# johnomotani/SharedMemSparseLU.jl

Measured on AMD Instinct MI355X. Metric: nnz(L+U)/s + achieved HBM GB/s, 3D Poisson 128³ numeric LU, 1/2/4/8 GPU, higher is better.
Workload: dtype f64

## Files before the change

### sharedmemsparselu.jl_amd/csrc/kernels_gemm.hip

```cpp
#include "kernels_common.hpp"

namespace smlu {

__device__ __forceinline__ int find_gemm_task(const GemmTask* __restrict__ t, int cnt, int64_t b) {
  int lo = 0, hi = cnt - 1;
  while (lo < hi) {
    int mid = (lo + hi + 1) >> 1;
    if (t[mid].tile0 <= b) lo = mid;
    else hi = mid - 1;
  }
  return lo;
}


__device__ __forceinline__ int64_t xcd_remap(int64_t b, int64_t nwg) {
  const int64_t q = nwg >> 3, r = nwg & 7, x = b & 7;
  return (x < r ? x * (q + 1) : r * (q + 1) + (x - r) * q) + (b >> 3);
}
__device__ __forceinline__ int64_t xcd_window_remap(int64_t b, int64_t nwg) {
  constexpr int64_t W = 512;
  if (b >= (nwg / W) * W) return b;
  const int64_t w0 = b - b % W, i = b % W;
  return w0 + (i & 7) * (W / 8) + (i >> 3);
}
template <int TS>
__device__ __forceinline__ void tile_rc(const GemmTask& t, int64_t tl, int& tm, int& tn) {
  constexpr int GM = 8;
  const int64_t tiles_n = (t.n + TS - 1) / TS;
  const int64_t g = tl / (GM * tiles_n);
  const int first = (int)(g * GM);
  const int gm = min(GM, t.tiles_m - first);
  const int64_t in = tl - g * GM * tiles_n;
  tm = first + (int)(in % gm);
  tn = (int)(in / gm);
}

struct GrowthArgs {
  int32_t* info;
  double* growth;
  double piv_tol;
};
__device__ __forceinline__ void tile_growth(const GrowthArgs& ga, int sid, double g) {
  g = wave_max(g);
  if ((threadIdx.x & 63) == 0 && g > 0.0) {
    atomic_max_pos(&ga.growth[0], g);
    if (g > 1.0 / ga.piv_tol) atomicOr(&ga.info[sid], 2);
  }
}

#define GBM 64
#define GBN 64
#define GBK 16
template <bool TRSM>
__global__ __launch_bounds__(256) void k_gemm(const GemmTask* __restrict__ tasks, int ntask, GrowthArgs ga) {
  __shared__ double As[2][GBK][GBM + 2];
  __shared__ double Bs[2][GBK][GBN + 2];
  const int64_t b = xcd_remap(blockIdx.x, gridDim.x);
  const GemmTask t = tasks[find_gemm_task(tasks, ntask, b)];
  const gdbl* gA = gbl(t.A);
  const gdbl* gB = gbl(t.B);
  gdbl* gC = gbl(t.C);
  int tm, tn;
  tile_rc<GBM>(t, b - t.tile0, tm, tn);
  const int m0 = tm * GBM, n0 = tn * GBN;
  const int tid = threadIdx.x;
  const int tx = tid & 15, ty = tid >> 4;
  double acc[4][4];
#pragma unroll
  for (int j = 0; j < 4; ++j) {
    const int col = n0 + ty + 16 * j;
#pragma unroll
    for (int i = 0; i < 4; ++i) {
      const int row = m0 + tx + 16 * i;
      acc[i][j] = (col < t.n && row < t.m) ? gC[(int64_t)col * t.ldc + row] : 0.0;
    }
  }
  const int ar = tid & 63, ak = tid >> 6;
  const int bk = tid & 15, bc = tid >> 4;
  double ra[4], rb[4];
  const int K = t.k;
  auto gload = [&](int k0) {
#pragma unroll
    for (int r = 0; r < 4; ++r) {
      int kk = ak + 4 * r;
      int row = m0 + ar;
      ra[r] = (row < t.m && k0 + kk < K) ? gA[(int64_t)(k0 + kk) * t.lda + row] : 0.0;
      int col = n0 + bc + 16 * r;
      rb[r] = (col < t.n && k0 + bk < K) ? gB[(int64_t)col * t.ldb + k0 + bk] : 0.0;
    }
  };
  auto sstore = [&](int buf) {
#pragma unroll
    for (int r = 0; r < 4; ++r) {
      As[buf][ak + 4 * r][ar] = ra[r];
      Bs[buf][bk][bc + 16 * r] = -rb[r];
    }
  };
  int nk = (K + GBK - 1) / GBK;
  gload(0);
  sstore(0);
  __syncthreads();
  for (int kt = 0; kt < nk; ++kt) {
    const int cur = kt & 1;
    if (kt + 1 < nk) gload((kt + 1) * GBK);
#pragma unroll 4
    for (int kk = 0; kk < GBK; ++kk) {
      double a[4], bb[4];
#pragma unroll
      for (int i = 0; i < 4; ++i) a[i] = As[cur][kk][tx + 16 * i];
#pragma unroll
      for (int j = 0; j < 4; ++j) bb[j] = Bs[cur][kk][ty + 16 * j];
#pragma unroll
      for (int i = 0; i < 4; ++i)
#pragma unroll
        for (int j = 0; j < 4; ++j) acc[i][j] = fma(a[i], bb[j], acc[i][j]);
    }
    if (kt + 1 < nk) sstore(cur ^ 1);
    __syncthreads();
  }
  double gmax = 0.0;
#pragma unroll
  for (int j = 0; j < 4; ++j) {
    const int col = n0 + ty + 16 * j;
#pragma unroll
    for (int i = 0; i < 4; ++i) {
      const int row = m0 + tx + 16 * i;
      if (col < t.n && row < t.m) {
        gC[(int64_t)col * t.ldc + row] = acc[i][j];
        gmax = fmax(gmax, fabs(acc[i][j]));
      }
    }
  }
  if (TRSM && t.gsid >= 0) tile_growth(ga, t.gsid, gmax);
}

typedef double v4d __attribute__((ext_vector_type(4)));
template <bool TRSM>
__global__ __launch_bounds__(256) void k_gemm64_mfma(const GemmTask* __restrict__ tasks, int ntask, GrowthArgs ga) {
  __shared__ double As[2][GBK][GBM + 2];
  __shared__ double Bs[2][GBK][GBN + 2];
  const int64_t b = xcd_remap(blockIdx.x, gridDim.x);
  const GemmTask t = tasks[find_gemm_task(tasks, ntask, b)];
  const gdbl* gA = gbl(t.A);
  const gdbl* gB = gbl(t.B);
  gdbl* gC = gbl(t.C);
  int tm, tn;
  tile_rc<GBM>(t, b - t.tile0, tm, tn);
  const int m0 = tm * GBM, n0 = tn * GBN;
  const int tid = threadIdx.x, lane = tid & 63;
  const int wv = __builtin_amdgcn_readfirstlane(tid >> 6);
  const int wr = (wv & 1) * 32, wc = (wv >> 1) * 32;
  const int li = lane & 15, lk = lane >> 4;
  v4d acc[2][2];
#pragma unroll
  for (int i = 0; i < 2; ++i) {
    const int row = m0 + wr + 16 * i + li;
#pragma unroll
    for (int j = 0; j < 2; ++j)
#pragma unroll
      for (int r = 0; r < 4; ++r) {
        const int col = n0 + wc + 16 * j + lk + 4 * r;
        acc[i][j][r] = (col < t.n && row < t.m) ? gC[(int64_t)col * t.ldc + row] : 0.0;
      }
  }
  const int ar = tid & 63, ak = tid >> 6;
  const int bk = tid & 15, bc = tid >> 4;
  double ra[4], rb[4];
  const int K = t.k;
  auto gload = [&](int k0) {
#pragma unroll
    for (int r = 0; r < 4; ++r) {
      const int kk = ak + 4 * r;
      const int row = m0 + ar;
      ra[r] = (row < t.m && k0 + kk < K) ? gA[(int64_t)(k0 + kk) * t.lda + row] : 0.0;
      const int col = n0 + bc + 16 * r;
      rb[r] = (col < t.n && k0 + bk < K) ? gB[(int64_t)col * t.ldb + k0 + bk] : 0.0;
    }
  };
  auto sstore = [&](int buf) {
#pragma unroll
    for (int r = 0; r < 4; ++r) {
      As[buf][ak + 4 * r][ar] = ra[r];
      Bs[buf][bk][bc + 16 * r] = -rb[r];
    }
  };
  const int nk = (K + GBK - 1) / GBK;
  gload(0);
  sstore(0);
  __syncthreads();
  for (int kt = 0; kt < nk; ++kt) {
    const int cur = kt & 1;
    if (kt + 1 < nk) gload((kt + 1) * GBK);
#pragma unroll
    for (int kq = 0; kq < GBK / 4; ++kq) {
      const int k = 4 * kq + lk;
      double fa[2], fb[2];
#pragma unroll
      for (int i = 0; i < 2; ++i) fa[i] = As[cur][k][wr + 16 * i + li];
#pragma unroll
      for (int j = 0; j < 2; ++j) fb[j] = Bs[cur][k][wc + 16 * j + li];
#pragma unroll
      for (int i = 0; i < 2; ++i)
#pragma unroll
        for (int j = 0; j < 2; ++j) acc[i][j] = __builtin_amdgcn_mfma_f64_16x16x4f64(fb[j], fa[i], acc[i][j], 0, 0, 0);
    }
    if (kt + 1 < nk) sstore(cur ^ 1);
    __syncthreads();
  }
  double gmax = 0.0;
#pragma unroll
  for (int i = 0; i < 2; ++i) {
    const int row = m0 + wr + 16 * i + li;
#pragma unroll
    for (int j = 0; j < 2; ++j)
#pragma unroll
      for (int r = 0; r < 4; ++r) {
        const int col = n0 + wc + 16 * j + lk + 4 * r;
        if (col < t.n && row < t.m) {
          gC[(int64_t)col * t.ldc + row] = acc[i][j][r];
          gmax = fmax(gmax, fabs(acc[i][j][r]));
        }
      }
  }
  if (TRSM && t.gsid >= 0) tile_growth(ga, t.gsid, gmax);
}

__device__ __forceinline__ double k64_tile_mfma(const gdbl* gA, int lda, const gdbl* gB, int ldb, gdbl* gC, int ldc,
                                                int m, int n, int K, int m0, int n0,
                                                double (&As)[64][GBM + 2], double (&Bs)[64][GBN + 2]) {
  const int tid = threadIdx.x, lane = tid & 63;
  const int wv = __builtin_amdgcn_readfirstlane(tid >> 6);
  const int wr = (wv & 1) * 32, wc = (wv >> 1) * 32;
  const int li = lane & 15, lk = lane >> 4;
  v4d acc[2][2];
#pragma unroll
  for (int i = 0; i < 2; ++i) {
    const int row = m0 + wr + 16 * i + li;
#pragma unroll
    for (int j = 0; j < 2; ++j)
#pragma unroll
      for (int r = 0; r < 4; ++r) {
        const int col = n0 + wc + 16 * j + lk + 4 * r;
        acc[i][j][r] = (col < n && row < m) ? gC[(int64_t)col * ldc + row] : 0.0;
      }
  }
  const int ar = tid & 63, ak = tid >> 6;
  double ra[16], rb[16];
#pragma unroll
  for (int r = 0; r < 16; ++r) {
    const int kk = ak + 4 * r, row = m0 + ar;
    ra[r] = (row < m && kk < K) ? gA[(int64_t)kk * lda + row] : 0.0;
    const int col = n0 + ak + 4 * r;
    rb[r] = (col < n && ar < K) ? gB[(int64_t)col * ldb + ar] : 0.0;
  }
#pragma unroll
  for (int r = 0; r < 16; ++r) {
    As[ak + 4 * r][ar] = ra[r];
    Bs[ar][ak + 4 * r] = -rb[r];
  }
  __syncthreads();
  auto kquad = [&](int kq) {
    const int k = 4 * kq + lk;
    double fa[2], fb[2];
#pragma unroll
    for (int i = 0; i < 2; ++i) fa[i] = As[k][wr + 16 * i + li];
#pragma unroll
    for (int j = 0; j < 2; ++j) fb[j] = Bs[k][wc + 16 * j + li];
#pragma unroll
    for (int i = 0; i < 2; ++i)
#pragma unroll
      for (int j = 0; j < 2; ++j) acc[i][j] = __builtin_amdgcn_mfma_f64_16x16x4f64(fb[j], fa[i], acc[i][j], 0, 0, 0);
  };
  if (K == 64) {
#pragma unroll
    for (int kq = 0; kq < 16; ++kq) kquad(kq);
  } else {
    const int nkq = (K + 3) >> 2;
    for (int kq = 0; kq < nkq; ++kq) kquad(kq);
  }
  double gmax = 0.0;
#pragma unroll
  for (int i = 0; i < 2; ++i) {
    const int row = m0 + wr + 16 * i + li;
#pragma unroll
    for (int j = 0; j < 2; ++j)
#pragma unroll
      for (int r = 0; r < 4; ++r) {
        const int col = n0 + wc + 16 * j + lk + 4 * r;
        if (col < n && row < m) {
          gC[(int64_t)col * ldc + row] = acc[i][j][r];
          gmax = fmax(gmax, fabs(acc[i][j][r]));
        }
      }
  }
  return gmax;
}

template <bool TRSM>
__global__ __launch_bounds__(256) void k_gemm_k64(const GemmTask* __restrict__ tasks, int ntask, GrowthArgs ga) {
  __shared__ double As[64][GBM + 2];
  __shared__ double Bs[64][GBN + 2];
  const int64_t b = xcd_remap(blockIdx.x, gridDim.x);
  const GemmTask t = tasks[find_gemm_task(tasks, ntask, b)];
  int tm, tn;
  tile_rc<GBM>(t, b - t.tile0, tm, tn);
  const double gmax = k64_tile_mfma(gbl(t.A), t.lda, gbl(t.B), t.ldb, gbl(t.C), t.ldc, t.m, t.n, t.k, tm * GBM,
                                    tn * GBN, As, Bs);
  if (TRSM && t.gsid >= 0) tile_growth(ga, t.gsid, gmax);
}

#define HBM_ 128
#define HBK_ 16
#define HLDB_ (HBM_ + 2)
__device__ __forceinline__ double sel0(bool c, double x) {
  return __longlong_as_double(__double_as_longlong(x) & (c ? -1LL : 0LL));
}
struct GatherArgs {
  const F22Gather* tg;
  const F22Child* ch;
  const int32_t* inv;
  const double* scratch;
};
struct F22Tile {
  const F22Child* ch;
  const int32_t* inv;
  const double* scratch;
  int cnt;
};
__device__ __forceinline__ double f22_child_val(const char* src, int nuc, int ri, int cj) {
  const bool ok = (ri | cj) >= 0;
  const uint32_t off = ok ? ((uint32_t)cj * (uint32_t)nuc + (uint32_t)ri) * 8u : 0u;
  return sel0(ok, *(const gdbl*)(src + off));
}
__device__ __forceinline__ void f22_child_add(v4d (&acc)[4][4], int j, const char* src, int nuc, const int (&ri)[4],
                                              const int (&cj)[4]) {
  double v[4][4];
#pragma unroll
  for (int r = 0; r < 4; ++r)
#pragma unroll
    for (int i = 0; i < 4; ++i) v[i][r] = f22_child_val(src, nuc, ri[i], cj[r]);
#pragma unroll
  for (int r = 0; r < 4; ++r)
#pragma unroll
    for (int i = 0; i < 4; ++i) acc[i][j][r] += v[i][r];
  __builtin_amdgcn_sched_barrier(0);
}
template <bool TRSM, bool FULL, bool GATHER = false>
__device__ __forceinline__ void gemm128_mfma_body(const GemmTask& t, int m0, int n0,
                                                double (&As)[2][HBK_][HBM_], double (&Bs)[2][HBK_][HLDB_],
                                                const GrowthArgs& ga, const F22Tile& fg = F22Tile{}) {
  const gdbl* gA = gbl(t.A);
  const gdbl* gB = gbl(t.B);
  gdbl* gC = gbl(t.C);
  const int tid = threadIdx.x, lane = tid & 63, wv = tid >> 6;
  const int wr = (wv & 1) * 64, wc = (wv >> 1) * 64;
  const int li = lane & 15, lk = lane >> 4;
  v4d acc[4][4];
  if (GATHER && fg.cnt >= 0) {
#pragma unroll
    for (int i = 0; i < 4; ++i)
#pragma unroll
      for (int j = 0; j < 4; ++j) acc[i][j] = v4d{0.0, 0.0, 0.0, 0.0};
#pragma unroll 1
    for (int d = 0; d < fg.cnt; ++d) {
      const F22Child c = fg.ch[d];
      if (c.hi < m0 + wr || c.lo >= m0 + wr + 64 || c.hi < n0 + wc || c.lo >= n0 + wc + 64) continue;
      const int32_t* inv = fg.inv + c.inv;
      const char* src = reinterpret_cast<const char*>(fg.scratch + c.foff);
      int ri[4], cj[4][4];
#pragma unroll
      for (int i = 0; i < 4; ++i) {
        const int row = m0 + wr + 16 * i + li;
        const int v = inv[min(row, t.m - 1)];
        ri[i] = row < t.m ? v : -1;
      }
#pragma unroll
      for (int j = 0; j < 4; ++j)
#pragma unroll
        for (int r = 0; r < 4; ++r) {
          const int col = n0 + wc + 16 * j + lk + 4 * r;
          const int v = inv[min(col, t.n - 1)];
          cj[j][r] = col < t.n ? v : -1;
        }
      __builtin_amdgcn_sched_barrier(0);
#pragma unroll
      for (int j = 0; j < 4; ++j) f22_child_add(acc, j, src, c.nu, ri, cj[j]);
    }
  } else {
#pragma unroll
    for (int i = 0; i < 4; ++i) {
      const int row = m0 + wr + 16 * i + li;
#pragma unroll
      for (int j = 0; j < 4; ++j)
#pragma unroll
        for (int r = 0; r < 4; ++r) {
          const int col = n0 + wc + 16 * j + lk + 4 * r;
          acc[i][j][r] = (FULL || (row < t.m && col < t.n)) ? gC[(int64_t)col * t.ldc + row] : 0.0;
        }
    }
  }
  const int ar = tid & 127, ak = tid >> 7;
  const int bk = tid & 15, bc = tid >> 4;
  const int K = t.k;
  const int arow = m0 + ar;
  const bool arow_ok = FULL || arow < t.m;
  const gdbl* Ap = gA + arow;
  const gdbl* Bp = gB + (int64_t)(n0 + bc) * t.ldb + bk;
  double ra[8], rb[8];
  auto gload = [&](int k0, bool kguard) {
#pragma unroll
    for (int r = 0; r < 8; ++r) {
      const int kk = k0 + ak + 2 * r;
      if (!kguard && FULL) ra[r] = Ap[(int64_t)kk * t.lda];
      else ra[r] = (arow_ok && kk < K) ? Ap[(int64_t)kk * t.lda] : 0.0;
      const int col = n0 + bc + 16 * r;
      if (!kguard && FULL) rb[r] = Bp[(int64_t)16 * r * t.ldb + k0];
      else rb[r] = ((FULL || col < t.n) && k0 + bk < K) ? Bp[(int64_t)16 * r * t.ldb + k0] : 0.0;
    }
  };
  auto sstore = [&](int buf) {
#pragma unroll
    for (int r = 0; r < 8; ++r) {
      As[buf][ak + 2 * r][ar] = ra[r];
      Bs[buf][bk][bc + 16 * r] = -rb[r];
    }
  };
  const int nk = (K + HBK_ - 1) / HBK_;
  const int nfull = K / HBK_;
  gload(0, nfull == 0);
  sstore(0);
  __syncthreads();
  for (int kt = 0; kt < nk; ++kt) {
    const int cur = kt & 1;
    if (kt + 1 < nk) gload((kt + 1) * HBK_, kt + 1 >= nfull);
#pragma unroll
    for (int kq = 0; kq < HBK_ / 4; ++kq) {
      const int k = kq * 4 + lk;
      double fa[4], fb[4];
#pragma unroll
      for (int i = 0; i < 4; ++i) fa[i] = As[cur][k][wr + 16 * i + li];
#pragma unroll
      for (int j = 0; j < 4; ++j) fb[j] = Bs[cur][k][wc + 16 * j + li];
#pragma unroll
      for (int i = 0; i < 4; ++i)
#pragma unroll
        for (int j = 0; j < 4; ++j)
          acc[i][j] = __builtin_amdgcn_mfma_f64_16x16x4f64(fb[j], fa[i], acc[i][j], 0, 0, 0);
    }
    if (kt + 1 < nk) sstore(cur ^ 1);
    __syncthreads();
  }
  double gmax = 0.0;
#pragma unroll
  for (int i = 0; i < 4; ++i) {
    const int row = m0 + wr + 16 * i + li;
#pragma unroll
    for (int j = 0; j < 4; ++j)
#pragma unroll
      for (int r = 0; r < 4; ++r) {
        const int col = n0 + wc + 16 * j + lk + 4 * r;
        if (FULL || (row < t.m && col < t.n)) {
          gC[(int64_t)col * t.ldc + row] = acc[i][j][r];
          if (TRSM) gmax = fmax(gmax, fabs(acc[i][j][r]));
        }
      }
  }
  if (TRSM && t.gsid >= 0) tile_growth(ga, t.gsid, gmax);
}


typedef double v2du __attribute__((ext_vector_type(2), aligned(8)));
typedef double v2d __attribute__((ext_vector_type(2)));
__device__ __forceinline__ v2d ldu2(const char* ubase, uint32_t off) {
  return *(const __attribute__((address_space(1))) v2du*)(ubase + off);
}
__device__ __forceinline__ void stu2(char* ubase, uint32_t off, v2d v) {
  *(__attribute__((address_space(1))) v2du*)(ubase + off) = v;
}

struct Mfma3Lds {
  double A[2][HBK_][HBM_];
  double B[2][HBM_][HBK_];
};
static_assert(sizeof(Mfma3Lds) == 65536, "v3 tile LDS image");
typedef __attribute__((address_space(3))) void lds_void;

__device__ __forceinline__ void glds16(const void* src, void* lds_dst) {
  __builtin_amdgcn_global_load_lds((const __attribute__((address_space(1))) void*)src, (lds_void*)lds_dst, 16, 0, 0);
}


template <bool TRSM, bool EB, bool GATHER = false>
__device__ __forceinline__ void gemm128_mfma3_interior(const GemmTask& t, int m0, int n0, Mfma3Lds& S,
                                                       const GrowthArgs& ga, const F22Tile& fg = F22Tile{}) {
  const int tid = threadIdx.x, lane = tid & 63;
  const int wv = __builtin_amdgcn_readfirstlane(tid >> 6);
  const int wr = (wv & 1) * 64, wc = (wv >> 1) * 64;
  const int li = lane & 15, lk = lane >> 4;
  const int K = t.k;
  const int64_t lda = t.lda, ldb = t.ldb, ldc = t.ldc;
  const uint32_t c_lo = (uint32_t)(((int64_t)lk * ldc + 2 * li) * 8);
  auto cbase = [&](int ip, int j, int r) {
    return reinterpret_cast<char*>(t.C) + ((int64_t)(n0 + wc + 16 * j + 4 * r) * ldc + m0 + wr + 32 * ip) * 8;
  };
  const int bpair = (lane & 7) ^ ((4 * wv + (lane >> 4)) & 7);
  const char* asrc = reinterpret_cast<const char*>(t.A) + ((int64_t)wv * lda + m0 + 2 * lane) * 8;
  const char* bsrc = reinterpret_cast<const char*>(t.B) + ((int64_t)(n0 + 8 * wv + (lane >> 3)) * ldb + 2 * bpair) * 8;
  auto issue = [&](int k0, int buf) {
#pragma unroll
    for (int q = 0; q < 4; ++q) {
      glds16(asrc + ((int64_t)(k0 + 4 * q) * lda) * 8, &S.A[buf][wv + 4 * q][0]);
      glds16(bsrc + ((int64_t)32 * q * ldb + k0) * 8, &S.B[buf][8 * (wv + 4 * q)][0]);
    }
  };
  auto stage_tail = [&](int k0, int buf) {
#pragma unroll
    for (int q = 0; q < 4; ++q) {
      const int ka = k0 + wv + 4 * q;
      const v2d a = ka < K ? ldu2(asrc + ((int64_t)(k0 + 4 * q) * lda) * 8, 0) : v2d{0.0, 0.0};
      *reinterpret_cast<v2d*>(&S.A[buf][wv + 4 * q][2 * lane]) = a;
      const gdbl* bp = gbl(reinterpret_cast<const double*>(bsrc + ((int64_t)32 * q * ldb + k0) * 8));
      const int kb = k0 + 2 * bpair;
      v2d b;
      b.x = kb < K ? bp[0] : 0.0;
      b.y = kb + 1 < K ? bp[1] : 0.0;
      *reinterpret_cast<v2d*>(&S.B[buf][8 * (wv + 4 * q)][2 * lane]) = b;
    }
  };
  v4d acc[4][4];
  if (GATHER && fg.cnt >= 0) {
#pragma unroll
    for (int i = 0; i < 4; ++i)
#pragma unroll
      for (int j = 0; j < 4; ++j) acc[i][j] = v4d{0.0, 0.0, 0.0, 0.0};
#pragma unroll 1
    for (int d = 0; d < fg.cnt; ++d) {
      const F22Child c = fg.ch[d];
      if (c.hi < m0 + wr || c.lo >= m0 + wr + 64 || c.hi < n0 + wc || c.lo >= n0 + wc + 64) continue;
      const int32_t* inv = fg.inv + c.inv;
      const char* src = reinterpret_cast<const char*>(fg.scratch + c.foff);
      int ri[4], cj[4][4];
#pragma unroll
      for (int ip = 0; ip < 2; ++ip) {
        ri[2 * ip] = inv[m0 + wr + 32 * ip + 2 * li];
        ri[2 * ip + 1] = inv[m0 + wr + 32 * ip + 2 * li + 1];
      }
#pragma unroll
      for (int j = 0; j < 4; ++j)
#pragma unroll
        for (int r = 0; r < 4; ++r) cj[j][r] = inv[n0 + wc + 16 * j + lk + 4 * r];
      __builtin_amdgcn_sched_barrier(0);
#pragma unroll
      for (int j = 0; j < 4; ++j) f22_child_add(acc, j, src, c.nu, ri, cj[j]);
    }
  } else {
#pragma unroll
    for (int ip = 0; ip < 2; ++ip)
#pragma unroll
      for (int j = 0; j < 4; ++j)
#pragma unroll
        for (int r = 0; r < 4; ++r) {
          const v2d c = ldu2(cbase(ip, j, r), c_lo);
          acc[2 * ip][j][r] = c.x;
          acc[2 * ip + 1][j][r] = c.y;
        }
  }
  const int a_off = (lk * HBM_ + wr + 2 * li);
  int b_off[4];
#pragma unroll
  for (int kq = 0; kq < 4; ++kq) b_off[kq] = (wc + li) * HBK_ + (((2 * kq + (lk >> 1)) ^ (li >> 1)) << 1) + (lk & 1);
  auto frags = [&](int cur, int kq, v2d (&fa)[2], double (&fb)[4]) {
    const double* As = &S.A[cur][0][0] + a_off + kq * 4 * HBM_;
    const double* Bs = &S.B[cur][0][0] + b_off[kq];
#pragma unroll
    for (int ip = 0; ip < 2; ++ip) fa[ip] = *reinterpret_cast<const v2d*>(As + 32 * ip);
#pragma unroll
    for (int j = 0; j < 4; ++j) fb[j] = Bs[16 * HBK_ * j];
  };
  auto quad = [&](const v2d (&fa)[2], const double (&fb)[4]) {
#pragma unroll
    for (int ip = 0; ip < 2; ++ip)
#pragma unroll
      for (int j = 0; j < 4; ++j) {
        acc[2 * ip][j] = __builtin_amdgcn_mfma_f64_16x16x4f64(fb[j], fa[ip].x, acc[2 * ip][j], 0, 0, 1);
        acc[2 * ip + 1][j] = __builtin_amdgcn_mfma_f64_16x16x4f64(fb[j], fa[ip].y, acc[2 * ip + 1][j], 0, 0, 1);
      }
  };
  auto slice = [&](int cur) {
    v2d fa0[2], fa1[2];
    double fb0[4], fb1[4];
    frags(cur, 0, fa0, fb0);
    frags(cur, 1, fa1, fb1);
    quad(fa0, fb0);
    frags(cur, 2, fa0, fb0);
    quad(fa1, fb1);
    frags(cur, 3, fa1, fb1);
    quad(fa0, fb0);
    quad(fa1, fb1);
  };
  const int nk = (K + HBK_ - 1) / HBK_;
  const int nfull = K / HBK_;
  if (nfull > 0) issue(0, 0);
  else stage_tail(0, 0);
  __syncthreads();
  if (!EB) {
    for (int kt = 0; kt < nk; ++kt) {
      const int cur = kt & 1;
      const bool next = kt + 1 < nk;
      const bool next_full = kt + 1 < nfull;
      if (next_full) issue((kt + 1) * HBK_, cur ^ 1);
      if (next && !next_full) stage_tail((kt + 1) * HBK_, cur ^ 1);
      slice(cur);
      if (next) __syncthreads();
    }
  } else {
    v2d fa0[2], fa1[2];
    double fb0[4], fb1[4];
    frags(0, 0, fa0, fb0);
    for (int kt = 0; kt < nk; ++kt) {
      const int cur = kt & 1;
      const bool next = kt + 1 < nk;
      const bool next_full = kt + 1 < nfull;
      if (next_full) issue((kt + 1) * HBK_, cur ^ 1);
      if (next && !next_full) stage_tail((kt + 1) * HBK_, cur ^ 1);
      frags(cur, 1, fa1, fb1);
      quad(fa0, fb0);
      frags(cur, 2, fa0, fb0);
      quad(fa1, fb1);
      frags(cur, 3, fa1, fb1);
      quad(fa0, fb0);
      if (next) {
        __syncthreads();
        frags(cur ^ 1, 0, fa0, fb0);
      }
      quad(fa1, fb1);
    }
  }
  double gmax = 0.0;
#pragma unroll
  for (int ip = 0; ip < 2; ++ip)
#pragma unroll
    for (int j = 0; j < 4; ++j)
#pragma unroll
      for (int r = 0; r < 4; ++r) {
        const v2d c = v2d{acc[2 * ip][j][r], acc[2 * ip + 1][j][r]};
        stu2(cbase(ip, j, r), c_lo, c);
        if (TRSM) gmax = fmax(gmax, fmax(fabs(c.x), fabs(c.y)));
      }
  if (TRSM && t.gsid >= 0) tile_growth(ga, t.gsid, gmax);
}

#ifdef SMLU_CLOCK_PROBE
__device__ unsigned long long* g_clock_probe = nullptr;
struct ClockMark {
  unsigned long long t0, r0;
  __device__ __forceinline__ ClockMark() : t0(__builtin_amdgcn_s_memtime()), r0(__builtin_amdgcn_s_memrealtime()) {}
  __device__ __forceinline__ void done(int form) const {
    const unsigned long long t1 = __builtin_amdgcn_s_memtime(), r1 = __builtin_amdgcn_s_memrealtime();
    unsigned long long* p = g_clock_probe;
    if (p && threadIdx.x == 0) {
      atomicAdd(p + 4 * form, t1 - t0);
      atomicAdd(p + 4 * form + 1, r1 - r0);
      atomicAdd(p + 4 * form + 2, 1ull);
    }
  }
};
#endif
template <bool TRSM, bool EB = false, bool GATHER = false>
__global__ __launch_bounds__(256, 2) void k_gemm128_mfma3(const GemmTask* __restrict__ tasks, int ntask,
                                                          GrowthArgs ga, GatherArgs gx) {
#ifdef SMLU_CLOCK_PROBE
  const ClockMark mark;
#endif
  __shared__ __attribute__((aligned(16))) double lds[sizeof(Mfma3Lds) / sizeof(double)];
  const int64_t b = xcd_window_remap(blockIdx.x, gridDim.x);
  const int ti = find_gemm_task(tasks, ntask, b);
  const GemmTask t = tasks[ti];
  F22Tile fg{nullptr, nullptr, nullptr, -1};
  if (GATHER) {
    const F22Gather g = gx.tg[ti];
    fg = F22Tile{gx.ch + g.beg, gx.inv, gx.scratch, g.cnt};
  }
  int tm, tn;
  tile_rc<HBM_>(t, b - t.tile0, tm, tn);
  const int m0 = tm * HBM_, n0 = tn * HBM_;
  if (m0 + HBM_ <= t.m && n0 + HBM_ <= t.n) {
    gemm128_mfma3_interior<TRSM, EB, GATHER>(t, m0, n0, *reinterpret_cast<Mfma3Lds*>(lds), ga, fg);
  } else {
    auto& As = *reinterpret_cast<double(*)[2][HBK_][HBM_]>(lds);
    auto& Bs = *reinterpret_cast<double(*)[2][HBK_][HLDB_]>(lds + 2 * HBK_ * HBM_);
    gemm128_mfma_body<TRSM, false, GATHER>(t, m0, n0, As, Bs, ga, fg);
  }
#ifdef SMLU_CLOCK_PROBE
  mark.done(EB ? 0 : 1);
#endif
}

#define UR_NC 32
#define UR_RB 6
#define UR_LD 36
__global__ __launch_bounds__(256, 2) void k_urows(const URowTask* __restrict__ tasks, const SNode* __restrict__ sn,
                                                  double* __restrict__ store, const double* __restrict__ tinv) {
  __shared__ double Bs[64 * UR_LD];
  const URowTask t = tasks[blockIdx.x];
  const SNode s = sn[t.s];
  const int64_t M = (int64_t)s.ns + s.nu;
  const int64_t ld = t.ld;
  const int nc = t.ncols;
  const int nrows = t.ob1 - t.ob0;
  const int tid = threadIdx.x, lane = tid & 63, li = lane & 15, lk = lane >> 4;
  const int wv = __builtin_amdgcn_readfirstlane(tid >> 6);
  gdbl* const C = gbl(store + t.coff);
  const gdbl* const Lp = gbl(store + s.Loff);
  v4d acc[UR_RB][2];
#pragma unroll
  for (int i = 0; i < UR_RB; ++i) {
    const int lr = 16 * (wv + 4 * i) + li;
    const bool rin = lr < nrows;
    const int row = t.ob0 + (rin ? lr : 0);
#pragma unroll
    for (int cb = 0; cb < 2; ++cb)
#pragma unroll
      for (int r = 0; r < 4; ++r) {
        const int col = 16 * cb + lk + 4 * r;
        const bool in = rin && col < nc;
        acc[i][cb][r] = sel0(in, C[(int64_t)(in ? col : 0) * ld + row]);
      }
  }
  auto publish = [&](int i) {
#pragma unroll
    for (int cb = 0; cb < 2; ++cb)
#pragma unroll
      for (int r = 0; r < 4; ++r) Bs[(16 * wv + li) * UR_LD + 16 * cb + lk + 4 * r] = -acc[i][cb][r];
  };
  const int nsub = (nrows + 63) >> 6;
#pragma unroll 1
  for (int u = 0; u < nsub; ++u) {
    const int kbu = t.ob0 + 64 * u;
    const int wu = min(64, t.ob1 - kbu);
    const int nkq = (wu + 3) >> 2;
    v4d tc[2];
#pragma unroll
    for (int i = 0; i < UR_RB; ++i)
      if (i == u) {
        publish(i);
        tc[0] = acc[i][0];
        tc[1] = acc[i][1];
      }
    double na[16];
    {
      const gdbl* pn = gbl(tinv + (int64_t)(t.slot0 + u) * 8192) + lk * 64 + 16 * wv + li;
#pragma unroll
      for (int kq = 0; kq < 16; ++kq) na[kq] = sel0(16 * wv + li < wu && 4 * kq + lk < wu, pn[256 * kq]);
    }
    __syncthreads();
#pragma unroll
    for (int kq = 0; kq < 16; ++kq) {
      if (kq >= nkq) continue;
      const int k = 4 * kq + lk;
#pragma unroll
      for (int cb = 0; cb < 2; ++cb)
        tc[cb] = __builtin_amdgcn_mfma_f64_16x16x4f64(Bs[k * UR_LD + 16 * cb + li], na[kq], tc[cb], 0, 0, 0);
    }
    __syncthreads();
#pragma unroll
    for (int i = 0; i < UR_RB; ++i)
      if (i == u) {
        acc[i][0] = tc[0];
        acc[i][1] = tc[1];
        publish(i);
      }
    __syncthreads();
    double fa[16], fn[16];
    auto lfrag = [&](int i, double (&f)[16]) {
      const int lr = 16 * (wv + 4 * i) + li;
      const bool rin = lr < nrows;
      const gdbl* pa = Lp + (int64_t)(kbu + lk) * M + t.ob0 + (rin ? lr : 0);
#pragma unroll
      for (int kq = 0; kq < 16; ++kq) {
        const bool kin = 4 * kq + lk < wu;
        f[kq] = sel0(rin && kin, pa[kin ? (int64_t)4 * kq * M : 0]);
      }
    };
    if (u + 1 < UR_RB && 16 * (wv + 4 * (u + 1)) < nrows) lfrag(u + 1, fa);
#pragma unroll
    for (int i = 1; i < UR_RB; ++i) {
      if (i <= u || 16 * (wv + 4 * i) >= nrows) continue;
      const bool more = i + 1 < UR_RB && 16 * (wv + 4 * (i + 1)) < nrows;
      if (more) lfrag(i + 1, fn);
#pragma unroll
      for (int kq = 0; kq < 16; ++kq) {
        if (kq >= nkq) continue;
        const int k = 4 * kq + lk;
#pragma unroll
        for (int cb = 0; cb < 2; ++cb)
          acc[i][cb] = __builtin_amdgcn_mfma_f64_16x16x4f64(Bs[k * UR_LD + 16 * cb + li], fa[kq], acc[i][cb], 0, 0, 0);
      }
      if (more)
#pragma unroll
        for (int kq = 0; kq < 16; ++kq) fa[kq] = fn[kq];
    }
    __syncthreads();
  }
#pragma unroll
  for (int i = 0; i < UR_RB; ++i) {
    const int lr = 16 * (wv + 4 * i) + li;
    if (16 * (wv + 4 * i) >= nrows) continue;
#pragma unroll
    for (int cb = 0; cb < 2; ++cb)
#pragma unroll
      for (int r = 0; r < 4; ++r) {
        const int col = 16 * cb + lk + 4 * r;
        if (lr < nrows && col < nc) C[(int64_t)col * ld + t.ob0 + lr] = acc[i][cb][r];
      }
  }
}

__global__ __launch_bounds__(256) void k_tri_inv(const int32_t* __restrict__ list, int step,
                                                 const SNode* __restrict__ sn,
                                                 double* __restrict__ store,
                                                 double* __restrict__ scratch,
                                                 double* __restrict__ tinv) {
  __shared__ double sD[64 * 65];
  const int item = blockIdx.x >> 3, part = blockIdx.x & 7;
  const int sid = list[2 * item];
  const int64_t slot = list[2 * item + 1];
  const SNode s = sn[sid];
  FrontPtrs f = front_ptrs(s, store, scratch);
  const int64_t M = f.M;
  const int kb = step * s.nb;
  const int w = min(s.nb, (int)f.ns - kb);
  const gdbl* D = f.L + (int64_t)kb * M + kb;
  {
    double v[16];
#pragma unroll
    for (int u = 0; u < 16; ++u) {
      const int idx = threadIdx.x + 256 * u, i = idx & 63, j = idx >> 6;
      v[u] = (i < w && j < w) ? D[(int64_t)j * M + i] : (i == j ? 1.0 : 0.0);
    }
#pragma unroll
    for (int u = 0; u < 16; ++u) {
      const int idx = threadIdx.x + 256 * u, i = idx & 63, j = idx >> 6;
      sD[j * 65 + i] = v[u];
    }
  }
  __syncthreads();
  const int lane = threadIdx.x & 63, wv = threadIdx.x >> 6;
  const bool upper = part >= 4;
  const int c0 = ((part & 3) * 4 + wv) * 4;
  double z[4];
#pragma unroll
  for (int r = 0; r < 4; ++r) z[r] = lane == c0 + r ? 1.0 : 0.0;
  double* out = tinv + slot * 8192 + (upper ? 4096 : 0);
  if (!upper) {
#pragma unroll 4
    for (int j = 0; j < 63; ++j) {
      const double lij = sD[j * 65 + lane];
#pragma unroll
      for (int r = 0; r < 4; ++r) {
        const double zj = readlane_f64(z[r], j);
        if (lane > j) z[r] = fma(-lij, zj, z[r]);
      }
    }
#pragma unroll
    for (int r = 0; r < 4; ++r) out[(int64_t)(c0 + r) * 64 + lane] = lane > c0 + r ? -z[r] : 0.0;
  } else {
    const double rd = recip(sD[lane * 65 + lane]);
#pragma unroll 4
    for (int j = 63; j >= 0; --j) {
      const double uij = sD[j * 65 + lane];
#pragma unroll
      for (int r = 0; r < 4; ++r) {
        if (lane == j) z[r] *= rd;
        const double yj = readlane_f64(z[r], j);
        if (lane < j) z[r] = fma(-uij, yj, z[r]);
      }
    }
#pragma unroll
    for (int r = 0; r < 4; ++r) {
      const int c = c0 + r;
      out[(int64_t)c * 64 + lane] = lane == c ? 1.0 - z[r] : (lane < c ? -z[r] : 0.0);
    }
  }
}

#ifdef SMLU_CLOCK_PROBE
extern "C" int smlu_dev_gemm_clock(int arm, unsigned long long* out) {
  static unsigned long long* buf = nullptr;
  if (!buf && hipMalloc(&buf, 8 * sizeof(unsigned long long)) != hipSuccess) return -1;
  unsigned long long* p = nullptr;
  if (arm) {
    if (hipMemset(buf, 0, 8 * sizeof(unsigned long long)) != hipSuccess) return -1;
    p = buf;
  } else {
    if (hipDeviceSynchronize() != hipSuccess) return -1;
    if (out && hipMemcpy(out, buf, 8 * sizeof(unsigned long long), hipMemcpyDeviceToHost) != hipSuccess) return -1;
  }
  return hipMemcpyToSymbol(HIP_SYMBOL(g_clock_probe), &p, sizeof p) == hipSuccess ? 0 : -1;
}
#endif

hipError_t launch_gemm_g(hipStream_t st, int64_t ntiles, const GemmTask* tasks, int ntask, int tile,
                         int64_t maxwg, int32_t* info, double* growth, double piv_tol) {
  if (ntiles <= 0) return hipSuccess;
  const GrowthArgs ga{info, growth, piv_tol};
  const GatherArgs gx{nullptr, nullptr, nullptr, nullptr};
  const bool trsm = info != nullptr;
  if (tile == 143) return hipErrorInvalidValue;
  if (tile == 135 && trsm) k_gemm128_mfma3<true, true><<<(unsigned)ntiles, 256, 0, st>>>(tasks, ntask, ga, gx);
  else if (tile == 135) k_gemm128_mfma3<false, true><<<(unsigned)ntiles, 256, 0, st>>>(tasks, ntask, ga, gx);
  else if (tile == 131 && trsm) k_gemm128_mfma3<true><<<(unsigned)ntiles, 256, 0, st>>>(tasks, ntask, ga, gx);
  else if (tile == 131) k_gemm128_mfma3<false><<<(unsigned)ntiles, 256, 0, st>>>(tasks, ntask, ga, gx);
  else if (tile == 65 && trsm) k_gemm_k64<true><<<(unsigned)ntiles, 256, 0, st>>>(tasks, ntask, ga);
  else if (tile == 65) k_gemm_k64<false><<<(unsigned)ntiles, 256, 0, st>>>(tasks, ntask, ga);
  else if (tile == 66 && trsm) k_gemm64_mfma<true><<<(unsigned)ntiles, 256, 0, st>>>(tasks, ntask, ga);
  else if (tile == 66) k_gemm64_mfma<false><<<(unsigned)ntiles, 256, 0, st>>>(tasks, ntask, ga);
  else if (trsm) k_gemm<true><<<(unsigned)ntiles, 256, 0, st>>>(tasks, ntask, ga);
  else k_gemm<false><<<(unsigned)ntiles, 256, 0, st>>>(tasks, ntask, ga);
  return hipGetLastError();
}
hipError_t launch_gemm(hipStream_t st, int64_t ntiles, const GemmTask* tasks, int ntask, int tile,
                       int64_t maxwg) {
  return launch_gemm_g(st, ntiles, tasks, ntask, tile, maxwg, nullptr, nullptr, 1.0);
}
hipError_t launch_gemm_gather(hipStream_t st, int64_t ntiles, const GemmTask* tasks, int ntask, const F22Gather* tg,
                              const F22Child* ch, const int32_t* inv, const double* scratch) {
  if (ntiles <= 0) return hipSuccess;
  if (!tg || !scratch) return hipErrorInvalidValue;
  const GrowthArgs ga{nullptr, nullptr, 1.0};
  const GatherArgs gx{tg, ch, inv, scratch};
  k_gemm128_mfma3<false, true, true><<<(unsigned)ntiles, 256, 0, st>>>(tasks, ntask, ga, gx);
  return hipGetLastError();
}
hipError_t launch_urows(hipStream_t st, int cnt, const URowTask* tasks, const SNode* sn, double* store,
                        const double* tinv) {
  if (cnt <= 0) return hipSuccess;
  k_urows<<<(unsigned)cnt, 256, 0, st>>>(tasks, sn, store, tinv);
  return hipGetLastError();
}
hipError_t launch_tri_inv(hipStream_t st, int cnt, int step, const int32_t* list, const SNode* sn,
                          double* store, double* scratch, double* tinv) {
  if (cnt <= 0) return hipSuccess;
  k_tri_inv<<<(unsigned)cnt * 8, 256, 0, st>>>(list, step, sn, store, scratch, tinv);
  return hipGetLastError();
}

}
```

Before: 6.558 billion.

## Replace edge-tile GEMM path with async-LDS mfma3 edge kernel and shape-specialized wave layouts

Partial (edge) 128x128 tiles no longer use the older register-staged gemm128_mfma_body. They now go through a new edge variant of the mfma3 interior path. That variant uses direct global-to-LDS loads when possible, a swizzled B layout, paired-row v2d loads and stores, and skips MFMAs for dead sub-tiles. Four template layouts redistribute the four waves depending on whether the remaining rows or columns exceed 64, so small edge tiles keep more waves busy. The cost is more code, more template instances and more complex boundary clamping, which may raise register pressure or add correctness risk at odd sizes.

```diff
diff --git a/sharedmemsparselu.jl_amd/csrc/kernels_gemm.hip b/sharedmemsparselu.jl_amd/csrc/kernels_gemm.hip
--- a/sharedmemsparselu.jl_amd/csrc/kernels_gemm.hip
+++ b/sharedmemsparselu.jl_amd/csrc/kernels_gemm.hip
@@ -311,7 +311,6 @@
 
 #define HBM_ 128
 #define HBK_ 16
-#define HLDB_ (HBM_ + 2)
 __device__ __forceinline__ double sel0(bool c, double x) {
   return __longlong_as_double(__double_as_longlong(x) & (c ? -1LL : 0LL));
 }
@@ -332,142 +331,20 @@
   const uint32_t off = ok ? ((uint32_t)cj * (uint32_t)nuc + (uint32_t)ri) * 8u : 0u;
   return sel0(ok, *(const gdbl*)(src + off));
 }
-__device__ __forceinline__ void f22_child_add(v4d (&acc)[4][4], int j, const char* src, int nuc, const int (&ri)[4],
+template <int NI, int NJ>
+__device__ __forceinline__ void f22_child_add(v4d (&acc)[NI][NJ], int j, const char* src, int nuc, const int (&ri)[NI],
                                               const int (&cj)[4]) {
-  double v[4][4];
+  double v[NI][4];
 #pragma unroll
   for (int r = 0; r < 4; ++r)
 #pragma unroll
-    for (int i = 0; i < 4; ++i) v[i][r] = f22_child_val(src, nuc, ri[i], cj[r]);
+    for (int i = 0; i < NI; ++i) v[i][r] = f22_child_val(src, nuc, ri[i], cj[r]);
 #pragma unroll
   for (int r = 0; r < 4; ++r)
 #pragma unroll
-    for (int i = 0; i < 4; ++i) acc[i][j][r] += v[i][r];
+    for (int i = 0; i < NI; ++i) acc[i][j][r] += v[i][r];
   __builtin_amdgcn_sched_barrier(0);
 }
-template <bool TRSM, bool FULL, bool GATHER = false>
-__device__ __forceinline__ void gemm128_mfma_body(const GemmTask& t, int m0, int n0,
-                                                double (&As)[2][HBK_][HBM_], double (&Bs)[2][HBK_][HLDB_],
-                                                const GrowthArgs& ga, const F22Tile& fg = F22Tile{}) {
-  const gdbl* gA = gbl(t.A);
-  const gdbl* gB = gbl(t.B);
-  gdbl* gC = gbl(t.C);
-  const int tid = threadIdx.x, lane = tid & 63, wv = tid >> 6;
-  const int wr = (wv & 1) * 64, wc = (wv >> 1) * 64;
-  const int li = lane & 15, lk = lane >> 4;
-  v4d acc[4][4];
-  if (GATHER && fg.cnt >= 0) {
-#pragma unroll
-    for (int i = 0; i < 4; ++i)
-#pragma unroll
-      for (int j = 0; j < 4; ++j) acc[i][j] = v4d{0.0, 0.0, 0.0, 0.0};
-#pragma unroll 1
-    for (int d = 0; d < fg.cnt; ++d) {
-      const F22Child c = fg.ch[d];
-      if (c.hi < m0 + wr || c.lo >= m0 + wr + 64 || c.hi < n0 + wc || c.lo >= n0 + wc + 64) continue;
-      const int32_t* inv = fg.inv + c.inv;
-      const char* src = reinterpret_cast<const char*>(fg.scratch + c.foff);
-      int ri[4], cj[4][4];
-#pragma unroll
-      for (int i = 0; i < 4; ++i) {
-        const int row = m0 + wr + 16 * i + li;
-        const int v = inv[min(row, t.m - 1)];
-        ri[i] = row < t.m ? v : -1;
-      }
-#pragma unroll
-      for (int j = 0; j < 4; ++j)
-#pragma unroll
-        for (int r = 0; r < 4; ++r) {
-          const int col = n0 + wc + 16 * j + lk + 4 * r;
-          const int v = inv[min(col, t.n - 1)];
-          cj[j][r] = col < t.n ? v : -1;
-        }
-      __builtin_amdgcn_sched_barrier(0);
-#pragma unroll
-      for (int j = 0; j < 4; ++j) f22_child_add(acc, j, src, c.nu, ri, cj[j]);
-    }
-  } else {
-#pragma unroll
-    for (int i = 0; i < 4; ++i) {
-      const int row = m0 + wr + 16 * i + li;
-#pragma unroll
-      for (int j = 0; j < 4; ++j)
-#pragma unroll
-        for (int r = 0; r < 4; ++r) {
-          const int col = n0 + wc + 16 * j + lk + 4 * r;
-          acc[i][j][r] = (FULL || (row < t.m && col < t.n)) ? gC[(int64_t)col * t.ldc + row] : 0.0;
-        }
-    }
-  }
-  const int ar = tid & 127, ak = tid >> 7;
-  const int bk = tid & 15, bc = tid >> 4;
-  const int K = t.k;
-  const int arow = m0 + ar;
-  const bool arow_ok = FULL || arow < t.m;
-  const gdbl* Ap = gA + arow;
-  const gdbl* Bp = gB + (int64_t)(n0 + bc) * t.ldb + bk;
-  double ra[8], rb[8];
-  auto gload = [&](int k0, bool kguard) {
-#pragma unroll
-    for (int r = 0; r < 8; ++r) {
-      const int kk = k0 + ak + 2 * r;
-      if (!kguard && FULL) ra[r] = Ap[(int64_t)kk * t.lda];
-      else ra[r] = (arow_ok && kk < K) ? Ap[(int64_t)kk * t.lda] : 0.0;
-      const int col = n0 + bc + 16 * r;
-      if (!kguard && FULL) rb[r] = Bp[(int64_t)16 * r * t.ldb + k0];
-      else rb[r] = ((FULL || col < t.n) && k0 + bk < K) ? Bp[(int64_t)16 * r * t.ldb + k0] : 0.0;
-    }
-  };
-  auto sstore = [&](int buf) {
-#pragma unroll
-    for (int r = 0; r < 8; ++r) {
-      As[buf][ak + 2 * r][ar] = ra[r];
-      Bs[buf][bk][bc + 16 * r] = -rb[r];
-    }
-  };
-  const int nk = (K + HBK_ - 1) / HBK_;
-  const int nfull = K / HBK_;
-  gload(0, nfull == 0);
-  sstore(0);
-  __syncthreads();
-  for (int kt = 0; kt < nk; ++kt) {
-    const int cur = kt & 1;
-    if (kt + 1 < nk) gload((kt + 1) * HBK_, kt + 1 >= nfull);
-#pragma unroll
-    for (int kq = 0; kq < HBK_ / 4; ++kq) {
-      const int k = kq * 4 + lk;
-      double fa[4], fb[4];
-#pragma unroll
-      for (int i = 0; i < 4; ++i) fa[i] = As[cur][k][wr + 16 * i + li];
-#pragma unroll
-      for (int j = 0; j < 4; ++j) fb[j] = Bs[cur][k][wc + 16 * j + li];
-#pragma unroll
-      for (int i = 0; i < 4; ++i)
-#pragma unroll
-        for (int j = 0; j < 4; ++j)
-          acc[i][j] = __builtin_amdgcn_mfma_f64_16x16x4f64(fb[j], fa[i], acc[i][j], 0, 0, 0);
-    }
-    if (kt + 1 < nk) sstore(cur ^ 1);
-    __syncthreads();
-  }
-  double gmax = 0.0;
-#pragma unroll
-  for (int i = 0; i < 4; ++i) {
-    const int row = m0 + wr + 16 * i + li;
-#pragma unroll
-    for (int j = 0; j < 4; ++j)
-#pragma unroll
-      for (int r = 0; r < 4; ++r) {
-        const int col = n0 + wc + 16 * j + lk + 4 * r;
-        if (FULL || (row < t.m && col < t.n)) {
-          gC[(int64_t)col * t.ldc + row] = acc[i][j][r];
-          if (TRSM) gmax = fmax(gmax, fabs(acc[i][j][r]));
-        }
-      }
-  }
-  if (TRSM && t.gsid >= 0) tile_growth(ga, t.gsid, gmax);
-}
-
 
 typedef double v2du __attribute__((ext_vector_type(2), aligned(8)));
 typedef double v2d __attribute__((ext_vector_type(2)));
@@ -650,6 +527,201 @@
   if (TRSM && t.gsid >= 0) tile_growth(ga, t.gsid, gmax);
 }
 
+template <bool TRSM, bool GATHER, int LAYOUT>
+__device__ __forceinline__ void gemm128_mfma3_edge(const GemmTask& t, int m0, int n0, int lm, int ln, Mfma3Lds& S,
+                                                   const GrowthArgs& ga, const F22Tile& fg) {
+  constexpr int NIP = (LAYOUT == 0 || LAYOUT == 2) ? 2 : 1;
+  constexpr int NJ = (LAYOUT == 0 || LAYOUT == 1) ? 4 : 2;
+  constexpr int BQ = (LAYOUT == 0 || LAYOUT == 2) ? 4 : 2;
+  const int tid = threadIdx.x, lane = tid & 63;
+  const int wv = __builtin_amdgcn_readfirstlane(tid >> 6);
+  const int wr = LAYOUT == 0 ? (wv & 1) * 64 : LAYOUT == 1 ? wv * 32 : LAYOUT == 2 ? 0 : (wv & 1) * 32;
+  const int wc = LAYOUT == 0 ? (wv >> 1) * 64 : LAYOUT == 1 ? 0 : LAYOUT == 2 ? wv * 32 : (wv >> 1) * 32;
+  const int li = lane & 15, lk = lane >> 4;
+  const int K = t.k;
+  const int64_t lda = t.lda, ldb = t.ldb;
+  const uint32_t ldc = (uint32_t)t.ldc;
+  const int nipl = min(NIP, max(0, (lm - wr + 31) >> 5));
+  const int njl = min(NJ, max(0, (ln - wc + 15) >> 4));
+  const bool live = nipl > 0 && njl > 0;
+  char* cb = reinterpret_cast<char*>(t.C) + ((int64_t)n0 * t.ldc + m0) * 8;
+  v4d acc[2 * NIP][NJ];
+  if (GATHER && fg.cnt >= 0) {
+#pragma unroll
+    for (int i = 0; i < 2 * NIP; ++i)
+#pragma unroll
+      for (int j = 0; j < NJ; ++j) acc[i][j] = v4d{0.0, 0.0, 0.0, 0.0};
+    if (live) {
+#pragma unroll 1
+      for (int d = 0; d < fg.cnt; ++d) {
+        const F22Child c = fg.ch[d];
+        if (c.hi < m0 + wr || c.lo >= m0 + wr + 32 * nipl || c.hi < n0 + wc || c.lo >= n0 + wc + 16 * njl) continue;
+        const int32_t* inv = fg.inv + c.inv;
+        const char* src = reinterpret_cast<const char*>(fg.scratch + c.foff);
+        int ri[2 * NIP], cj[NJ][4];
+#pragma unroll
+        for (int i = 0; i < 2 * NIP; ++i) {
+          const int row = m0 + wr + 32 * (i >> 1) + 2 * li + (i & 1);
+          const int v = inv[min(row, t.m - 1)];
+          ri[i] = row < t.m ? v : -1;
+        }
+#pragma unroll
+        for (int j = 0; j < NJ; ++j)
+#pragma unroll
+          for (int r = 0; r < 4; ++r) {
+            const int col = n0 + wc + 16 * j + lk + 4 * r;
+            const int v = inv[min(col, t.n - 1)];
+            cj[j][r] = col < t.n ? v : -1;
+          }
+        __builtin_amdgcn_sched_barrier(0);
+#pragma unroll
+        for (int j = 0; j < NJ; ++j)
+          if (j < njl) f22_child_add(acc, j, src, c.nu, ri, cj[j]);
+      }
+    }
+  } else {
+#pragma unroll
+    for (int ip = 0; ip < NIP; ++ip) {
+      const int rl = wr + 32 * ip + 2 * li;
+      const int rc = min(rl, lm - 2);
+#pragma unroll
+      for (int j = 0; j < NJ; ++j)
+#pragma unroll
+        for (int r = 0; r < 4; ++r) {
+          const uint32_t cl = (uint32_t)min(wc + 16 * j + lk + 4 * r, ln - 1);
+          if (lm >= 2) {
+            const v2d c = ldu2(cb, (cl * ldc + (uint32_t)rc) * 8u);
+            acc[2 * ip][j][r] = rl > rc ? c.y : c.x;
+            acc[2 * ip + 1][j][r] = c.y;
+          } else {
+            acc[2 * ip][j][r] = acc[2 * ip + 1][j][r] = *(const gdbl*)(cb + cl * ldc * 8u);
+          }
+        }
+    }
+  }
+  const int bpair = (lane & 7) ^ ((4 * wv + (lane >> 4)) & 7);
+  const char* bbase = reinterpret_cast<const char*>(t.B) + ((int64_t)n0 * ldb + 2 * bpair) * 8;
+  auto bsrc = [&](int q, int k0) {
+    return bbase + ((int64_t)min(8 * (wv + 4 * q) + (lane >> 3), ln - 1) * ldb + k0) * 8;
+  };
+  const bool a_dma = lm == HBM_ || !(lm & 1);
+  const char* abase = reinterpret_cast<const char*>(t.A) + ((int64_t)wv * lda + m0) * 8;
+  const uint32_t a_pair = (uint32_t)max(min(2 * lane, lm - 2), 0) * 8u;
+  const uint32_t a_x = (uint32_t)min(2 * lane, lm - 1) * 8u, a_y = (uint32_t)min(2 * lane + 1, lm - 1) * 8u;
+  auto issue = [&](int k0, int buf) {
+#pragma unroll
+    for (int q = 0; q < 4; ++q) {
+      if (a_dma) glds16(abase + ((int64_t)(k0 + 4 * q) * lda) * 8 + a_pair, &S.A[buf][wv + 4 * q][0]);
+      if (q < BQ) glds16(bsrc(q, k0), &S.B[buf][8 * (wv + 4 * q)][0]);
+    }
+  };
+  auto tail_b = [&](int k0, int buf) {
+#pragma unroll
+    for (int q = 0; q < BQ; ++q) {
+      const gdbl* bp = gbl(reinterpret_cast<const double*>(bsrc(q, k0)));
+      const int kb = k0 + 2 * bpair;
+      v2d b;
+      b.x = kb < K ? bp[0] : 0.0;
+      b.y = kb + 1 < K ? bp[1] : 0.0;
+      *reinterpret_cast<v2d*>(&S.B[buf][8 * (wv + 4 * q)][2 * lane]) = b;
+    }
+  };
+  v2d areg[4];
+  auto load_a = [&](int k0) {
+#pragma unroll
+    for (int q = 0; q < 4; ++q) {
+      const char* p = abase + ((int64_t)(k0 + 4 * q) * lda) * 8;
+      if (k0 + wv + 4 * q < K) areg[q] = v2d{*(const gdbl*)(p + a_x), *(const gdbl*)(p + a_y)};
+      else areg[q] = v2d{0.0, 0.0};
+    }
+  };
+  auto store_a = [&](int buf) {
+#pragma unroll
+    for (int q = 0; q < 4; ++q) *reinterpret_cast<v2d*>(&S.A[buf][wv + 4 * q][2 * lane]) = areg[q];
+  };
+  const int a_off = (lk * HBM_ + wr + 2 * li);
+  int b_off[4];
+#pragma unroll
+  for (int kq = 0; kq < 4; ++kq) b_off[kq] = (wc + li) * HBK_ + (((2 * kq + (lk >> 1)) ^ (li >> 1)) << 1) + (lk & 1);
+  auto frags = [&](int cur, int kq, v2d (&fa)[NIP], double (&fb)[NJ]) {
+    const double* As = &S.A[cur][0][0] + a_off + kq * 4 * HBM_;
+    const double* Bs = &S.B[cur][0][0] + b_off[kq];
+#pragma unroll
+    for (int ip = 0; ip < NIP; ++ip) fa[ip] = *reinterpret_cast<const v2d*>(As + 32 * ip);
+#pragma unroll
+    for (int j = 0; j < NJ; ++j) fb[j] = Bs[16 * HBK_ * j];
+  };
+  auto quad = [&](const v2d (&fa)[NIP], const double (&fb)[NJ]) {
+#pragma unroll
+    for (int j = 0; j < NJ; ++j)
+      if (j < njl) {
+#pragma unroll
+        for (int ip = 0; ip < NIP; ++ip)
+          if (ip < nipl) {
+            acc[2 * ip][j] = __builtin_amdgcn_mfma_f64_16x16x4f64(fb[j], fa[ip].x, acc[2 * ip][j], 0, 0, 1);
+            acc[2 * ip + 1][j] = __builtin_amdgcn_mfma_f64_16x16x4f64(fb[j], fa[ip].y, acc[2 * ip + 1][j], 0, 0, 1);
+          }
+      }
+  };
+  auto slice = [&](int cur) {
+    v2d fa0[NIP], fa1[NIP];
+    double fb0[NJ], fb1[NJ];
+    frags(cur, 0, fa0, fb0);
+    frags(cur, 1, fa1, fb1);
+    quad(fa0, fb0);
+    frags(cur, 2, fa0, fb0);
+    quad(fa1, fb1);
+    frags(cur, 3, fa1, fb1);
+    quad(fa0, fb0);
+    quad(fa1, fb1);
+  };
+  const int nk = (K + HBK_ - 1) / HBK_;
+  const int nfull = K / HBK_;
+  if (nfull > 0) issue(0, 0);
+  else tail_b(0, 0);
+  if (!(a_dma && nfull > 0)) {
+    load_a(0);
+    store_a(0);
+  }
+  __syncthreads();
+  for (int kt = 0; kt < nk; ++kt) {
+    const int cur = kt & 1;
+    const bool next = kt + 1 < nk;
+    const bool next_full = kt + 1 < nfull;
+    const bool a_regs = next && !(a_dma && next_full);
+    if (next_full) issue((kt + 1) * HBK_, cur ^ 1);
+    if (next && !next_full) tail_b((kt + 1) * HBK_, cur ^ 1);
+    if (a_regs) load_a((kt + 1) * HBK_);
+    if (live) slice(cur);
+    if (a_regs) store_a(cur ^ 1);
+    if (next) __syncthreads();
+  }
+  double gmax = 0.0;
+#pragma unroll
+  for (int ip = 0; ip < NIP; ++ip)
+    if (ip < nipl) {
+      const int rl = wr + 32 * ip + 2 * li;
+#pragma unroll
+      for (int j = 0; j < NJ; ++j)
+        if (j < njl) {
+#pragma unroll
+          for (int r = 0; r < 4; ++r) {
+            const int cl = wc + 16 * j + lk + 4 * r;
+            const uint32_t off = ((uint32_t)cl * ldc + (uint32_t)rl) * 8u;
+            const double x = acc[2 * ip][j][r], y = acc[2 * ip + 1][j][r];
+            if (cl < ln && rl + 1 < lm) {
+              stu2(cb, off, v2d{x, y});
+              if (TRSM) gmax = fmax(gmax, fmax(fabs(x), fabs(y)));
+            } else if (cl < ln && rl < lm) {
+              *(gdbl*)(cb + off) = x;
+              if (TRSM) gmax = fmax(gmax, fabs(x));
+            }
+          }
+        }
+    }
+  if (TRSM && t.gsid >= 0) tile_growth(ga, t.gsid, gmax);
+}
+
 #ifdef SMLU_CLOCK_PROBE
 __device__ unsigned long long* g_clock_probe = nullptr;
 struct ClockMark {
@@ -687,9 +759,12 @@
   if (m0 + HBM_ <= t.m && n0 + HBM_ <= t.n) {
     gemm128_mfma3_interior<TRSM, EB, GATHER>(t, m0, n0, *reinterpret_cast<Mfma3Lds*>(lds), ga, fg);
   } else {
-    auto& As = *reinterpret_cast<double(*)[2][HBK_][HBM_]>(lds);
-    auto& Bs = *reinterpret_cast<double(*)[2][HBK_][HLDB_]>(lds + 2 * HBK_ * HBM_);
-    gemm128_mfma_body<TRSM, false, GATHER>(t, m0, n0, As, Bs, ga, fg);
+    Mfma3Lds& S = *reinterpret_cast<Mfma3Lds*>(lds);
+    const int lm = min(HBM_, t.m - m0), ln = min(HBM_, t.n - n0);
+    if (lm > 64 && ln > 64) gemm128_mfma3_edge<TRSM, GATHER, 0>(t, m0, n0, lm, ln, S, ga, fg);
+    else if (lm > 64) gemm128_mfma3_edge<TRSM, GATHER, 1>(t, m0, n0, lm, ln, S, ga, fg);
+    else if (ln > 64) gemm128_mfma3_edge<TRSM, GATHER, 2>(t, m0, n0, lm, ln, S, ga, fg);
+    else gemm128_mfma3_edge<TRSM, GATHER, 3>(t, m0, n0, lm, ln, S, ga, fg);
   }
 #ifdef SMLU_CLOCK_PROBE
   mark.done(EB ? 0 : 1);
```

Measured after the change: 6.671 billion, median of 6. +1.7%, better.
